# phazei/ComfyUI-HunyuanVideo-Foley

Hardware: AMD Instinct MI355X
Metric: audio-sec/sec (5s clip, 50-step Euler, CFG 4.5) (higher is better)
Workload: dtype bf16; 1 GPU; c2: T2A 5 s, 50 Euler steps, CFG 4.5, hunyuanvideo-foley-xxl, bs=1/GPU, bf16 GEMM operands / fp32 accumulate, weight storage none, DAC-VAE fp32 decode to 48 kHz, host-to-host (H2D noise + D2H waveform timed); clips_per_gpu=1, parallelism=dp1, hip_graph=True, progress_callback=False, collectives=0, bundle_bytes=10565004032, rccl_nranks=1

## Files before the change

comfyui-hunyuanvideo-foley_amd/csrc/foley_rt.hip:

```cpp
#include "../../include/foley_hip.h"
#include "kernels.h"
#include "gemm_plan.h"

#include <algorithm>
#include <climits>
#include <cmath>
#include <cstdio>
#include <cstdlib>
#include <cstring>
#include <cxxabi.h>
#include <atomic>
#include <mutex>
#include <string>
#include <unordered_map>
#include <vector>

thread_local FoleyProfHook g_foley_prof = {nullptr, nullptr};

static std::mutex g_setup_mutex;

static thread_local std::string g_err;
int foley_set_err(const char* msg, const char* file, int line) {
  const char* base = strrchr(file, '/');
  g_err = std::string(msg) + " (" + (base ? base + 1 : file) + ":" + std::to_string(line) + ")";
// ... 699 lines not shown
  RowBcast r{base, ld, 2, rows_per_cfg, L, nullptr, 0, Ls, (float)Ls / (float)L, per, 0, 0};
  if (per > 0) {
    r.dense_from = lead < 0 ? INT_MAX : lead;
    r.dense_base = lead < 0 ? 0 : lead * per;
  }
  return r;
}

static int prof_begin(foley_ctx* c, hipStream_t st, const char* label, double flop, double bytes) {
  if (!c->prof.on) return 0;
  ProfRec r{label, flop, bytes, c->prof.get(), c->prof.get(), nullptr};
  c->prof.recs.push_back(r);
  g_foley_prof = FoleyProfHook{r.e0, r.e1, nullptr};
  return 0;
}
static int prof_end(foley_ctx* c, hipStream_t st) {
  if (!c->prof.on) return 0;
  if (g_foley_prof.e0) {
    g_foley_prof.e0 = nullptr;
    HIPTRY(hipEventRecord(c->prof.recs.back().e0, st));
    HIPTRY(hipEventRecord(c->prof.recs.back().e1, st));
  } else {
    c->prof.recs.back().fn = g_foley_prof.fn;
  }
  return 0;
}
#define PROF(label, flop, bytes, call)            \
  do {                                            \
    TRY(prof_begin(c, st, (label), (flop), (bytes))); \
    TRY(call);                                    \
    TRY(prof_end(c, st));                         \
  } while (0)

static int run_forward(foley_ctx* c, hipStream_t st) {
  const foley_config& f = c->cfg;
  const foley_plan& pl = c->plan;
  const ForwardW& W = c->fw;
  if (!W.ok) return FAIL(FOLEY_ERR_STATE, "forward weights are not resolved (foley_prepare)");
  auto krot = [&pl](GemmArgs g) {
    g.krot_ok = pl.clips == 1 ? 1 : 0;
    return g;
  };
  const int D = f.hidden, H = f.heads, C = f.latent_dim, T = f.compute_dtype;
  const int ncfg = pl.ncfg, clips = pl.clips, La = pl.La, Lv = pl.Lv, Ls = pl.Ls, Lt = pl.Lt, NI = pl.n_iter;
  const int Bc = ncfg * clips, M = Bc * La, Mv = Bc * Lv, S = La + Lv;
  const int th = c->txt_rows ? Bc : ncfg, vh = c->vis_rows ? Bc : ncfg, tdiv = Bc / th, vdiv = Bc / vh;
  const bool bf = foley_is_half(T);
  const size_t es = esize(T);
  const int Sp = (S + 31) & ~31, Lap = (La + 31) & ~31;
  const int* sp = c->step_ctr;
  auto gf = [](double m, double n, double k) { return 2.0 * m * n * k; };
  auto gb = [&](double m, double n, double k, double out_es) { return (m * k + n * k) * (double)es + m * n * out_es; };
  auto af = [&](double b, double sq, double skv) { return 4.0 * b * H * sq * skv * 128.0; };
  auto ab = [&](double b, double sq, double skv) { return (2.0 * b * H * sq * 128.0 + 2.0 * b * H * skv * 128.0) * (double)es; };

  if (!c->smod_hoisted) {
    const int lead = c->sync_per ? c->sync_lead : 0, R = lead * c->sync_per + (vh - lead) * Ls;
    if (c->vis_rows && lead > 1)
      TRY(launch_rows_add_act(c->sync_lead_rows, rb_vec(c->vec_table, D, sp), lead * c->sync_per, D, 1, c->svec, T, st));
    else
      for (int h = 0; h < lead; ++h)
        TRY(launch_rows_add_act(c->sync_tok + (size_t)h * Ls * D, rb_vec(c->vec_table, D, sp), c->sync_per, D, 1,
                                (char*)c->svec + (size_t)h * c->sync_per * D * es, T, st));
    if (lead < vh)
      TRY(launch_rows_add_act(c->sync_tok + (size_t)lead * Ls * D, rb_vec(c->vec_table, D, sp), (vh - lead) * Ls, D, 1,
                              (char*)c->svec + (size_t)lead * c->sync_per * D * es, T, st));
    if (f.depth_single > 0) {
      const double n = (double)f.depth_single * 6 * D;
      GemmArgs gm = krot(gemm_plain(c->svec, R, W.smod, c->smod, (long)f.depth_single * 6 * D));
      PROF("single.modulation (all blocks, one GEMM)", gf(R, n, D), gb(R, n, D, 4), launch_gemm(gm, T, EPI_STORE_F32, 0, st));
    }
  }

  {
    GemmArgs g = krot(gemm_plain(c->xin, M, W.audio_in, c->audio, D));
    g.rb = rb_up(c->sync_tok, D, vdiv * La, La, Ls);
    PROF("audio_embedder", gf(M, D, C), gb(M, D, C, 4), launch_gemm(g, T, EPI_STORE_F32, 0, st));
  }
  if (c->vis_rows)
    TRY(launch_gather_rows(c->v_cond0, c->rep_idx, Bc * Lv, 1, c->vis_src * Lv, D, c->vcond, st));
  else
    TRY(launch_gather_rows(c->v_cond0, c->rep_idx, clips * Lv, ncfg, Lv, D, c->vcond, st));

  LnPending pend[2] = {LnPending{}, LnPending{}};
  const int slab_half = bf ? T : 0;
  auto with_partials = [&](GemmArgs& g, float* slabs) {
    g.partial_half = slab_half ? 1 : 0;
    g.partials = slabs;
    g.partial_stride = (long)g.M * g.N;
    g.partial_cap = PART_CAP;
  };
  const double ln_bytes_t = (double)(M + Mv) * D * (4 + 4 + es), ln_bytes_s = (double)M * D * (4 + 4 + es);
  for (int blk = 0; blk < f.depth_triple; ++blk) {
    const TripleW& w = W.t[blk];
    auto tb = [&](int s, int chunk) {
      return rb_vec(c->modtab + ((size_t)(blk * 2 + s) * NI) * 9 * D + (size_t)chunk * D, 9L * D, sp);
    };
    struct Stream { float* x; void* xn; float* qkv; void* att; void* hid; int rows, L, tok_off; const int* pos; };
    Stream ss[2] = {{c->audio, c->xn_a, c->qkv_a, c->att_a, c->hid_a, M, La, Lv, pl.pos_audio_self},
                    {c->vcond, c->xn_v, c->qkv_v, c->att_v, c->hid_v, Mv, Lv, 0, pl.pos_visual_self}};
    auto ln2 = [&](int c_shift, int c_scale) -> int {
      LnArgs a0{ss[0].x, ss[0].rows, tb(0, c_shift), tb(0, c_scale), ss[0].xn, pend[0]};
      LnArgs a1{ss[1].x, ss[1].rows, tb(1, c_shift), tb(1, c_scale), ss[1].xn, pend[1]};
      pend[0] = pend[1] = LnPending{};
      PROF("triple.layernorm+modulate (+pending split-K sum)", 0.0, ln_bytes_t, launch_ln_mod_pair(a0, a1, D, 1e-6f, T, st));
      return 0;
    };
    auto gated2 = [&](const char* label, const Lin& la, const Lin& lv, bool from_hid, int c_gate) -> int {
      GemmArgs g0 = krot(gemm_plain(from_hid ? ss[0].hid : ss[0].att, ss[0].rows, la, ss[0].x, D));
      GemmArgs g1 = krot(gemm_plain(from_hid ? ss[1].hid : ss[1].att, ss[1].rows, lv, ss[1].x, D));
      g0.rb = tb(0, c_gate);
      g1.rb = tb(1, c_gate);
      with_partials(g0, c->part_a);
      with_partials(g1, c->part_v);
      int ks = 1;
// ... 111 lines not shown
         launch_ln_mod_pending(c->audio, M, D, 1e-5f, sm(3), sm(4), c->xn_a, T, pend[0], st));
    pend[0] = LnPending{};
    PROF("single.w1/w3 conv3 GEMM + SiLU gate", gf(M, 2 * Hc, 3 * D), gb(M, 2 * Hc, 3 * D, es) - (double)M * Hc * es,
         launch_gemm(krot(gemm_conv(c->xn_a, M, La, D, 3, 1, w.w13, c->hid_a, Hc)), T, EPI_SILUGATE_T, 0, st));
    {
      GemmArgs g = krot(gemm_conv(c->hid_a, M, La, Hc, 3, 1, w.w2, c->audio, D));
      g.rb = sm(5);
      with_partials(g, c->part_a);
      int ks = 1;
      PROF("single.w2 conv3 GEMM (gated residual)", gf(M, D, 3 * Hc), gb(M, D, 3 * Hc, 4), launch_gemm(g, T, EPI_GATE_RES, 0, st, &ks));
      if (ks > 1) pend[0] = LnPending{c->part_a, ks, g.partial_stride, w.w2.b, g.rb, slab_half};
    }
  }

  {
    PROF("final.layernorm", 0.0, ln_bytes_s,
         launch_ln_mod_pending(c->audio, M, D, 1e-6f, rb_none(), rb_none(), c->xn_a, T, pend[0], st));
    PROF("final.linear", gf(M, C, D), gb(M, C, D, 4), launch_gemm(krot(gemm_plain(c->xn_a, M, W.fin, c->pred, C)), T, EPI_STORE_F32, 0, st));
  }
  return 0;
}

extern "C" int foley_dit_forward(foley_ctx* c, const float* latents, int iter, float* out_rows, void* stream_v) {
  if (!c || !latents || !out_rows) return FAIL(FOLEY_ERR_INVALID, "null argument");
  if (!c->prepared) return FAIL(FOLEY_ERR_STATE, "foley_prepare has not been called");
  if (iter < 0 || iter >= c->plan.n_iter) return FAIL(FOLEY_ERR_INVALID, "iteration out of range");
  hipStream_t st = (hipStream_t)stream_v;
  HIPTRY(hipSetDevice(c->device));
  const foley_plan& pl = c->plan;
  const int C = c->cfg.latent_dim;
  HIPTRY(hipMemcpyAsync(c->step_ctr, &iter, sizeof(int), hipMemcpyHostToDevice, st));
  HIPTRY(hipStreamSynchronize(st));
  TRY(launch_latent_rows(latents, pl.clips, C, pl.La, pl.ncfg, c->xin, c->cfg.compute_dtype, st));
  TRY(run_forward(c, st));
  HIPTRY(hipMemcpyAsync(out_rows, c->pred, (size_t)pl.ncfg * pl.clips * pl.La * C * 4, hipMemcpyDeviceToDevice, st));
  return 0;
}

extern "C" int foley_profile_forward(foley_ctx* c, const float* latents, int iter, int repeats, foley_prof_entry* out,
                                     int cap, int* n_out, float* bracket_ms, void* stream_v) {
  if (!c || !latents || !out || !n_out || cap < 1 || repeats < 1) return FAIL(FOLEY_ERR_INVALID, "bad argument");
  if (!c->prepared) return FAIL(FOLEY_ERR_STATE, "foley_prepare has not been called");
  if (iter < 0 || iter >= c->plan.n_iter) return FAIL(FOLEY_ERR_INVALID, "iteration out of range");
  hipStream_t st = (hipStream_t)stream_v;
  HIPTRY(hipSetDevice(c->device));
  const foley_plan& pl = c->plan;
  HIPTRY(hipMemcpyAsync(c->step_ctr, &iter, sizeof(int), hipMemcpyHostToDevice, st));
  HIPTRY(hipStreamSynchronize(st));
  TRY(launch_latent_rows(latents, pl.clips, c->cfg.latent_dim, pl.La, pl.ncfg, c->xin, c->cfg.compute_dtype, st));
  TRY(run_forward(c, st));
  c->prof.recs.clear();
  c->prof.used = 0;
  c->prof.on = true;
  int rc = 0;
  for (int r = 0; r < repeats && rc == 0; ++r) rc = run_forward(c, st);
  c->prof.on = false;
  g_foley_prof = FoleyProfHook{nullptr, nullptr, nullptr};
  if (rc) return rc;
  constexpr int NCAL = 32;
  hipEvent_t cal[2 * NCAL];
  for (int i = 0; i < 2 * NCAL; ++i) cal[i] = c->prof.get();
  for (int i = 0; i < NCAL; ++i) {
    HIPTRY(hipEventRecord(cal[2 * i], st));
    HIPTRY(hipEventRecord(cal[2 * i + 1], st));
  }
  HIPTRY(hipStreamSynchronize(st));
  double cal_ms = 0.0;
  for (int i = 0; i < NCAL; ++i) {
    float ms = 0.f;
    HIPTRY(hipEventElapsedTime(&ms, cal[2 * i], cal[2 * i + 1]));
    cal_ms += ms;
  }
  if (bracket_ms) *bracket_ms = (float)(cal_ms / NCAL);
  int n = 0;
  for (const ProfRec& r : c->prof.recs) {
    float ms = 0.f;
    HIPTRY(hipEventElapsedTime(&ms, r.e0, r.e1));
    int j = 0;
    for (; j < n; ++j)
      if (!strcmp(out[j].label, r.label)) break;
    if (j == n) {
      if (n == cap) return FAIL(FOLEY_ERR_INVALID, "profile: entry buffer too small");
      memset(&out[n], 0, sizeof(out[n]));
      strncpy(out[n].label, r.label, sizeof(out[n].label) - 1);
      if (r.fn) {
        const char* mangled = hipKernelNameRefByPtr(r.fn, st);
        if (mangled) {
          int status = 0;
          char* dm = abi::__cxa_demangle(mangled, nullptr, nullptr, &status);
          strncpy(out[n].kernel, status == 0 && dm ? dm : mangled, sizeof(out[n].kernel) - 1);
          free(dm);
        }
      }
      ++n;
    }
    out[j].calls += 1;
    out[j].total_ms += ms;
    out[j].flop += r.flop;
    out[j].bytes += r.bytes;
  }
  *n_out = n;
  return 0;
}

static int run_iteration(foley_ctx* c, hipStream_t st) {
  const foley_plan& pl = c->plan;
  TRY(run_forward(c, st));
  StepArgs s{};
  s.pred = c->pred; s.x = c->x_cur; s.x_saved = c->x_saved; s.d_acc = c->d_acc;
  s.clips = pl.clips; s.C = c->cfg.latent_dim; s.L = pl.La; s.ncfg = pl.ncfg;
  s.guidance = pl.guidance; s.coef = pl.solver_coef; s.step_ptr = c->step_ctr;
  s.rows_out = c->xin; s.rows_dtype = c->cfg.compute_dtype;
  if (c->edit) {
    StepEditArgs e{};
    e.s = s;
    e.x0 = (const float*)c->edit_x0.p; e.noise = (const float*)c->edit_noise.p;
    e.mask = c->edit_mask_clips ? (const float*)c->edit_mask.p : nullptr;
    e.x0_clips = c->edit_x0_clips; e.mask_clips = c->edit_mask_clips;
    return launch_solver_step_edit(e, st);
  }
  return launch_solver_step(s, st);
}

static int edit_key(const foley_ctx* c) {
  if (!c->edit) return 0;
  return 1 | (c->edit_x0_clips == 1 ? 2 : 0) | (c->edit_mask_clips ? 4 : 0) | (c->edit_mask_clips == 1 ? 8 : 0);
}

extern "C" int foley_set_edit(foley_ctx* c, const float* x0, int x0_clips, const float* noise, const float* mask, int mask_clips,
                              void* stream_v) {
  if (!c) return FAIL(FOLEY_ERR_INVALID, "null context");
  if (!c->prepared) return FAIL(FOLEY_ERR_STATE, "foley_set_edit: foley_prepare has not been called");
  if (!x0 && !noise && !mask) {
    c->edit = false;
    return 0;
  }
  if (!x0 || !noise) return FAIL(FOLEY_ERR_INVALID, "foley_set_edit: x0 and noise are required (all three null clears the edit state)");
  const foley_plan& pl = c->plan;
  if (x0_clips != 1 && x0_clips != pl.clips) return FAIL(FOLEY_ERR_INVALID, "foley_set_edit: x0_clips must be 1 or the plan's clips");
  if (mask && mask_clips != 1 && mask_clips != pl.clips)
    return FAIL(FOLEY_ERR_INVALID, "foley_set_edit: mask_clips must be 1 or the plan's clips");
  std::lock_guard<std::mutex> setup_lock(g_setup_mutex);
  hipStream_t st = (hipStream_t)stream_v;
  HIPTRY(hipSetDevice(c->device));
  HIPTRY(hipStreamSynchronize(st));
// ... 15 lines not shown
extern "C" int foley_sample(foley_ctx* c, float* latents, int use_graph, foley_progress_cb cb, void* user,
                            void* stream_v) {
  if (!c || !latents) return FAIL(FOLEY_ERR_INVALID, "null argument");
  if (!c->prepared) return FAIL(FOLEY_ERR_STATE, "foley_prepare has not been called");
  hipStream_t st = (hipStream_t)stream_v;
  HIPTRY(hipSetDevice(c->device));
  const foley_plan& pl = c->plan;
  const size_t xbytes = (size_t)pl.clips * c->cfg.latent_dim * pl.La * 4;
  if (c->graph_exec && c->graph_key != edit_key(c)) ctx_drop_graph(c);
  if (use_graph && !c->graph_exec) {
    std::lock_guard<std::mutex> setup_lock(g_setup_mutex);
    hipStream_t cs;
    HIPTRY(hipStreamSynchronize(st));
    HIPTRY(hipStreamCreateWithFlags(&cs, hipStreamNonBlocking));
    hipGraph_t graph = nullptr;
    hipError_t e = hipStreamBeginCapture(cs, hipStreamCaptureModeThreadLocal);
    int rc = 0;
    if (e == hipSuccess) {
      rc = run_iteration(c, cs);
      hipError_t e2 = hipStreamEndCapture(cs, &graph);
      if (e == hipSuccess) e = e2;
    }
    if (e == hipSuccess && rc == 0) e = hipGraphInstantiate(&c->graph_exec, graph, nullptr, nullptr, 0);
    if (graph) (void)hipGraphDestroy(graph);
    (void)hipStreamDestroy(cs);
    if (rc != 0) return rc;
    if (e != hipSuccess) return FAIL(FOLEY_ERR_HIP, hipGetErrorString(e));
    c->graph_guidance = pl.guidance;
    c->graph_key = edit_key(c);
  }
  c->abort_req.store(0, std::memory_order_relaxed);
  HIPTRY(hipEventRecord(c->ev0, st));
  HIPTRY(hipMemcpyAsync(c->x_cur, latents, xbytes, hipMemcpyDeviceToDevice, st));
  HIPTRY(hipMemsetAsync(c->step_ctr, 0, sizeof(int), st));
  TRY(launch_latent_rows(c->x_cur, pl.clips, c->cfg.latent_dim, pl.La, pl.ncfg, c->xin, c->cfg.compute_dtype, st));
  for (int it = 0; it < pl.n_iter; ++it) {
    if (use_graph) HIPTRY(hipGraphLaunch(c->graph_exec, st));
    else TRY(run_iteration(c, st));
    if (cb) {
      HIPTRY(hipMemcpyAsync(latents, c->x_cur, xbytes, hipMemcpyDeviceToDevice, st));
      HIPTRY(hipStreamSynchronize(st));
      cb(it + 1, pl.n_iter, user);
    }
    if (c->abort_req.exchange(0, std::memory_order_acq_rel)) {
      if (!cb) {
        HIPTRY(hipMemcpyAsync(latents, c->x_cur, xbytes, hipMemcpyDeviceToDevice, st));
        HIPTRY(hipStreamSynchronize(st));
      }
      return FAIL(FOLEY_ERR_ABORTED, "sampling loop aborted by foley_abort()");
    }
  }
  HIPTRY(hipMemcpyAsync(latents, c->x_cur, xbytes, hipMemcpyDeviceToDevice, st));
  HIPTRY(hipEventRecord(c->ev1, st));
  c->timed = true;
  return 0;
}

extern "C" int foley_abort(foley_ctx* c) {
  if (!c) return FAIL(FOLEY_ERR_INVALID, "null context");
  c->abort_req.store(1, std::memory_order_release);
  return 0;
}

extern "C" int foley_dac_decode(foley_ctx* c, const float* latents, int clips, int T, float* wave, void* stream_v) {
  if (!c || !latents || !wave || clips < 1 || T < 1) return FAIL(FOLEY_ERR_INVALID, "bad argument");
  hipStream_t st = (hipStream_t)stream_v;
  HIPTRY(hipSetDevice(c->device));
  const foley_config& f = c->cfg;
// ... 356 lines not shown
  for (int i = 0; i < 2; ++i) {
    if (a[i].M < 0) return FAIL(FOLEY_ERR_INVALID, "ln_mod pair: negative row count");
    if (!parts[i]) continue;
    if (ks[i] < 1 || !gate[i]) return FAIL(FOLEY_ERR_INVALID, "pending split-K: partials, k >= 1 and a gate are required");
    if (pdt[i] != 0 && pdt[i] != out_dtype) return FAIL(FOLEY_ERR_INVALID, "pending split-K: 16-bit slabs must have the output dtype");
    a[i].pend = LnPending{(const float*)parts[i], ks[i], (long)a[i].M * D, bias[i], to_rb(gate[i]), pdt[i]};
  }
  return launch_ln_mod_pair(a[0], a[1], D, eps, out_dtype, (hipStream_t)stream);
}

extern "C" int foley_op_ln_mod_pending(float* x, int M, int D, float eps, const foley_rowbcast* shift,
                                       const foley_rowbcast* scale, void* out, int out_dtype, const float* partials,
                                       int k, const float* bias, const foley_rowbcast* gate, void* stream) {
  return foley_op_ln_mod_pending2(x, M, D, eps, shift, scale, out, out_dtype, partials, 0, k, bias, gate, stream);
}

extern "C" int foley_op_qkv_split(const float* qkv, int M, int L, int H, int nK, const float* const* gain,
                                  const int32_t* const* pos, void* const* dst, int out_dtype, int vt_pitch,
                                  int S_tot, int tok_off, float eps, const float* cos_tab, const float* sin_tab,
                                  void* stream) {
  if (nK < 1 || nK > 3) return FAIL(FOLEY_ERR_INVALID, "nK must be 1..3");
  QkvSplitArgs a{};
  a.qkv = qkv; a.M = M; a.L = L; a.H = H; a.nK = nK;
  for (int i = 0; i < nK; ++i) {
    a.gain[i] = gain ? gain[i] : nullptr;
    a.pos[i] = pos ? pos[i] : nullptr;
    a.dst[i] = dst[i];
  }
  a.out_dtype = out_dtype; a.vt_pitch = vt_pitch;
  a.S_tot = S_tot; a.tok_off = tok_off; a.eps = eps; a.cos_tab = cos_tab; a.sin_tab = sin_tab;
  return launch_qkv_split(a, (hipStream_t)stream);
}

extern "C" int foley_op_solver_step(const float* pred, float* x, float* x_saved, float* d_acc, int clips, int C,
                                    int L, int ncfg, float guidance, const float* coef, int32_t* step_ptr,
                                    void* rows_out, int rows_dtype, void* stream) {
  StepArgs s{pred, x, x_saved, d_acc, clips, C, L, ncfg, guidance, coef, step_ptr, rows_out, rows_dtype};
  return launch_solver_step(s, (hipStream_t)stream);
}

extern "C" int foley_op_solver_step_edit(const float* pred, float* x, float* x_saved, float* d_acc, int clips, int C, int L,
                                         int ncfg, float guidance, const float* coef, int32_t* step_ptr, void* rows_out,
                                         int rows_dtype, const float* x0, int x0_clips, const float* noise, const float* mask,
                                         int mask_clips, void* stream) {
  StepEditArgs e{};
  e.s = StepArgs{pred, x, x_saved, d_acc, clips, C, L, ncfg, guidance, coef, step_ptr, rows_out, rows_dtype};
  e.x0 = x0; e.noise = noise; e.mask = mask; e.x0_clips = x0_clips; e.mask_clips = mask_clips;
  return launch_solver_step_edit(e, (hipStream_t)stream);
}

extern "C" int foley_op_flow_mix(const float* noise, const float* x0, int x0_clips, int clips, int C, int L, float sigma,
                                 float* out, void* stream) {
  return launch_flow_mix(noise, x0, x0_clips, clips, C, L, sigma, out, (hipStream_t)stream);
}

extern "C" int foley_op_latent_rows(const float* x, int clips, int C, int L, int ncfg, void* out, int out_dtype,
                                    void* stream) {
  return launch_latent_rows(x, clips, C, L, ncfg, out, out_dtype, (hipStream_t)stream);
}

extern "C" int foley_op_dac_out(const float* s, const float* w, const float* bias, int B, int T, int C, float* out,
                                void* stream) {
  return launch_dac_out(s, w, bias, B, T, C, out, (hipStream_t)stream);
}
```

comfyui-hunyuanvideo-foley_amd/csrc/kernels.h:

```cpp
#pragma once
#include "common.h"

enum GemmEpi {
  EPI_STORE_F32 = 0,
  EPI_STORE_T = 1,
  EPI_SILU_T = 2,
  EPI_GELU_T = 3,
  EPI_SILUGATE_T = 4,
  EPI_GATE_RES = 5,
  EPI_DAC = 6,
  EPI_QKV_SPLIT = 7,
  EPI_QKV_ATTN = 8,
  EPI_COUNT
};

struct QkvSplitArgs {
  const float* qkv;
  int M, L, H, nK;
  const float* gain[3];
  const int* pos[3];
  void* dst[3];
  int S_tot, tok_off;
  int out_dtype;
  int vt_pitch;
// ... 78 lines not shown
  const float* partials;
  int k;
  long stride;
  const float* bias;
  RowBcast gate;
  int half;
};
struct LnArgs {
  float* x;
  int M;
  RowBcast shift, scale;
  void* out;
  LnPending pend;
};
int launch_ln_mod_pending(float* x, int M, int D, float eps, const RowBcast& shift, const RowBcast& scale,
                          void* out, int out_dtype, const LnPending& pend, hipStream_t st);
int launch_ln_mod_pair(const LnArgs& a0, const LnArgs& a1, int D, float eps, int out_dtype, hipStream_t st);

int launch_qkv_split(const QkvSplitArgs& a, hipStream_t st);
int launch_qkv_split_pair(const QkvSplitArgs& a0, const QkvSplitArgs& a1, hipStream_t st);

int launch_rows_add_act(const float* a, const RowBcast& v, int R, int D, int act_silu, void* out,
                        int out_dtype, hipStream_t st);
int launch_rows_periodic_check(const float* x, int groups, int rows, int period, int D, int* flag, hipStream_t st);
int launch_add_periodic(const float* x, const float* pos, int R, int D, int period, void* out,
                        int out_dtype, hipStream_t st);
int launch_gather_rows(const float* src, const int* idx, int n_idx, int groups, int src_rows, int D,
                       float* out, hipStream_t st);
int launch_cast(const void* src, int src_dtype, void* dst, int dst_dtype, long n, hipStream_t st);

int launch_latent_rows(const float* x, int clips, int C, int L, int ncfg, void* out, int out_dtype,
                       hipStream_t st);

struct StepArgs {
  const float* pred;
  float* x;
  float* x_saved;
  float* d_acc;
  int clips, C, L, ncfg;
  float guidance;
  const float* coef;
  int* step_ptr;
  void* rows_out;
  int rows_dtype;
};
int launch_solver_step(const StepArgs& a, hipStream_t st);
struct StepEditArgs {
  StepArgs s;
  const float* x0;
  const float* noise;
  const float* mask;
  int x0_clips, mask_clips;
};
int launch_solver_step_edit(const StepEditArgs& a, hipStream_t st);
int launch_flow_mix(const float* noise, const float* x0, int x0_clips, int clips, int C, int L, float sigma, float* out,
                    hipStream_t st);

int launch_dac_in(const float* x, const float* w, const float* bias, const float* alpha, int B, int T, int C,
                  float* out0, float* out1, hipStream_t st);
int launch_rows_to_planes(const float* rows, int B, int T, int C, float* out, hipStream_t st);
int launch_qkv_regroup(const void* qkv, int n_rows, int dtype, int H, const int* idx_q, int G, int Sq, const int* idx_kv, int Skv, void* q, void* k,
                       void* v, int vt_pitch, hipStream_t st);
int launch_resize_aa_u8(const uint8_t* in, long outer, int len_in, long inner, int len_out, const int* xmin, const int* xsize,
                        const short* w, int kmax, int prec, uint8_t* out, hipStream_t st);
int launch_resample_sinc(const float* x, int B, int N, int orig, int nnew, const float* taps, int ntaps, int width, float* out,
                         int Nout, hipStream_t st);
int launch_logmel(const float* w16, int B, int N16, const float* basis, const int* mel_lo, const int* mel_len, const float* mel_w,
                  int mel_wp, void* patches, int out_dtype, float* mel_out, hipStream_t st);
int launch_dac_out(const float* s, const float* w, const float* bias, int B, int T, int C, float* out,
                   hipStream_t st);
```

comfyui-hunyuanvideo-foley_amd/csrc/rowops.hip:

```cpp
#include <type_traits>

#include "kernels.h"

namespace {

#define FOLEY_LAUNCH_CHECK()                                                             \
  do {                                                                                   \
    hipError_t _e = hipGetLastError();                                                   \
    if (_e != hipSuccess) return foley_set_err(hipGetErrorString(_e), __FILE__, __LINE__); \
  } while (0)

template <typename OutT> struct Pack4;
template <> struct Pack4<float> {
  static __device__ __forceinline__ void store(float* p, const f32x4 v) { *(f32x4*)p = v; }
};
template <> struct Pack4<bf16_t> {
  static __device__ __forceinline__ void store(bf16_t* p, const f32x4 v) {
    uint2 w;
    w.x = pack_bf16x2(v[0], v[1]);
    w.y = pack_bf16x2(v[2], v[3]);
    *(uint2*)p = w;
  }
};

template <> struct Pack4<f16_t> {
  static __device__ __forceinline__ void store(f16_t* p, const f32x4 v) {
    uint2 w;
    w.x = pack_f16x2(v[0], v[1]);
    w.y = pack_f16x2(v[2], v[3]);
    *(uint2*)p = w;
  }
};
// ... 353 lines not shown
    out[i] = src[((long)g * src_rows + idx[l]) * D + c];
  }
}

template <typename S, typename Dst>
__global__ void cast_kernel(const S* __restrict__ s, Dst* __restrict__ d, long n) {
  for (long i = (long)blockIdx.x * blockDim.x + threadIdx.x; i < n; i += (long)gridDim.x * blockDim.x)
    d[i] = Cvt<Dst>::to(Cvt<S>::from(s[i]));
}

template <typename OutT>
__global__ __launch_bounds__(256) void latent_rows_kernel(const float* __restrict__ x, int clips, int C, int L,
                                                          int ncfg, OutT* __restrict__ out) {
  __shared__ float tile[32][33];
  const int b = blockIdx.z;
  const int l0 = blockIdx.x * 32, c0 = blockIdx.y * 32;
  const int tx = threadIdx.x & 31, ty = threadIdx.x >> 5;
  for (int i = ty; i < 32; i += 8) {
    const int c = c0 + i, l = l0 + tx;
    tile[i][tx] = (c < C && l < L) ? x[((long)b * C + c) * L + l] : 0.f;
  }
  __syncthreads();
  for (int i = ty; i < 32; i += 8) {
    const int l = l0 + i, c = c0 + tx;
    if (l < L && c < C) {
      const OutT v = Cvt<OutT>::to(tile[tx][i]);
      for (int g = 0; g < ncfg; ++g) out[(((long)g * clips + b) * L + l) * C + c] = v;
    }
  }
}

constexpr int STEP_SAVE_X = 1, STEP_USE_SAVED = 2, STEP_ACC_RESET = 4;

template <typename OutT>
__global__ __launch_bounds__(256) void solver_step_kernel(const StepArgs a) {
  __shared__ float tile[32][33];
  const int it = *a.step_ptr;
  const float* cf = a.coef + (long)it * 8;
  const float w_new = cf[0], w_acc = cf[1], dt = cf[2], w_store = cf[3];
  const int flags = (int)cf[4];
  const int b = blockIdx.z;
  const int l0 = blockIdx.x * 32, c0 = blockIdx.y * 32;
  const int tx = threadIdx.x & 31, ty = threadIdx.x >> 5;
  const long rows = (long)a.clips * a.L;
  for (int i = ty; i < 32; i += 8) {
    const int l = l0 + i, c = c0 + tx;
    float v = 0.f;
    if (l < a.L && c < a.C) {
      const long r = (long)b * a.L + l;
      if (a.ncfg == 2) {
        const float u = a.pred[r * a.C + c], cnd = a.pred[(rows + r) * a.C + c];
        v = u + a.guidance * (cnd - u);
      } else {
        v = a.pred[r * a.C + c];
      }
    }
    tile[i][tx] = v;
  }
  __syncthreads();
  for (int i = ty; i < 32; i += 8) {
    const int c = c0 + i, l = l0 + tx;
    float xn = 0.f;
    if (c < a.C && l < a.L) {
      const long xi = ((long)b * a.C + c) * a.L + l;
      const float v = tile[tx][i];
      const float xc = a.x[xi];
      float acc = 0.f;
      if (a.d_acc) acc = (flags & STEP_ACC_RESET) ? 0.f : a.d_acc[xi];
      const float deriv = (w_acc != 0.f) ? (w_new * v + w_acc * acc) : (w_new * v);
      const float base = (flags & STEP_USE_SAVED) ? a.x_saved[xi] : xc;
      if (flags & STEP_SAVE_X) a.x_saved[xi] = xc;
      xn = base + deriv * dt;
      a.x[xi] = xn;
      if (a.d_acc) a.d_acc[xi] = acc + w_store * v;
    }
    tile[tx][i] = xn;
  }
  __syncthreads();
  if (a.rows_out) {
    for (int i = ty; i < 32; i += 8) {
      const int l = l0 + i, c = c0 + tx;
      if (l < a.L && c < a.C) {
        const OutT v = Cvt<OutT>::to(tile[i][tx]);
        for (int g = 0; g < a.ncfg; ++g)
          ((OutT*)a.rows_out)[(((long)g * a.clips + b) * a.L + l) * a.C + c] = v;
      }
    }
  }
}

constexpr int STEP_BLEND = 8;

template <typename OutT>
__global__ __launch_bounds__(256) void solver_step_edit_kernel(const StepEditArgs e) {
  __shared__ float tile[32][33];
  const StepArgs& a = e.s;
  const int it = *a.step_ptr;
  const float* cf = a.coef + (long)it * 8;
  const float w_new = cf[0], w_acc = cf[1], dt = cf[2], w_store = cf[3];
  const int flags = (int)cf[4];
  const float s_next = cf[5];
  const int b = blockIdx.z;
  const int l0 = blockIdx.x * 32, c0 = blockIdx.y * 32;
  const int tx = threadIdx.x & 31, ty = threadIdx.x >> 5;
  const long rows = (long)a.clips * a.L;
  for (int i = ty; i < 32; i += 8) {
    const int l = l0 + i, c = c0 + tx;
    float v = 0.f;
    if (l < a.L && c < a.C) {
      const long r = (long)b * a.L + l;
      if (a.ncfg == 2) {
        const float u = a.pred[r * a.C + c], cnd = a.pred[(rows + r) * a.C + c];
        v = u + a.guidance * (cnd - u);
      } else {
        v = a.pred[r * a.C + c];
      }
    }
    tile[i][tx] = v;
  }
  __syncthreads();
  const float* x0b = e.x0 + (e.x0_clips == 1 ? 0L : (long)b * a.C * a.L);
  const float* mb = e.mask ? e.mask + (e.mask_clips == 1 ? 0L : (long)b * a.L) : nullptr;
  for (int i = ty; i < 32; i += 8) {
    const int c = c0 + i, l = l0 + tx;
    float xn = 0.f;
    if (c < a.C && l < a.L) {
      const long xi = ((long)b * a.C + c) * a.L + l;
      const float v = tile[tx][i];
      const float xc = a.x[xi];
      float acc = 0.f;
      if (a.d_acc) acc = (flags & STEP_ACC_RESET) ? 0.f : a.d_acc[xi];
      const float deriv = (w_acc != 0.f) ? (w_new * v + w_acc * acc) : (w_new * v);
      const float base = (flags & STEP_USE_SAVED) ? a.x_saved[xi] : xc;
      if (flags & STEP_SAVE_X) a.x_saved[xi] = xc;
      xn = base + deriv * dt;
      if (flags & STEP_BLEND) {
        const float m = mb ? mb[l] : 1.f;
        const float tgt = s_next * e.noise[xi] + (1.f - s_next) * x0b[(long)c * a.L + l];
        xn = m * xn + (1.f - m) * tgt;
      }
      a.x[xi] = xn;
      if (a.d_acc) a.d_acc[xi] = acc + w_store * v;
    }
    tile[tx][i] = xn;
  }
  __syncthreads();
  if (a.rows_out) {
    for (int i = ty; i < 32; i += 8) {
      const int l = l0 + i, c = c0 + tx;
      if (l < a.L && c < a.C) {
        const OutT v = Cvt<OutT>::to(tile[i][tx]);
        for (int g = 0; g < a.ncfg; ++g)
          ((OutT*)a.rows_out)[(((long)g * a.clips + b) * a.L + l) * a.C + c] = v;
      }
    }
  }
}

__global__ __launch_bounds__(256) void flow_mix_kernel(const float* __restrict__ noise, const float* __restrict__ x0,
                                                       long plane, long n, int x0_per_clip, float sigma,
                                                       float* __restrict__ out) {
  const long i = (long)blockIdx.x * 256 + threadIdx.x;
  if (i >= n) return;
  const float src = x0[x0_per_clip ? i : i % plane];
  out[i] = sigma * noise[i] + (1.f - sigma) * src;
}

__global__ void step_increment_kernel(int* p) { *p = *p + 1; }

__global__ __launch_bounds__(256) void dac_out_kernel(const float* __restrict__ s, const float* __restrict__ w,
                                                      const float* __restrict__ bias, int T, int C,
                                                      float* __restrict__ out) {
  extern __shared__ float sm[];
  const int b = blockIdx.y;
  const int t0 = blockIdx.x * 64;
  const int pitch = C + 1;
  float* rows = sm;
  float* wl = sm + 70 * pitch;
  for (int i = threadIdx.x; i < 7 * C; i += 256) wl[i] = w[i];
  for (int i = threadIdx.x; i < 70 * C; i += 256) {
    const int rr = i / C, c = i - rr * C;
    const int t = t0 + rr - 3;
    rows[rr * pitch + c] = (t >= 0 && t < T) ? s[((long)b * T + t) * C + c] : 0.f;
  }
  __syncthreads();
  const int ti = threadIdx.x >> 2, part = threadIdx.x & 3;
  const int cq = C >> 2;
  float acc = 0.f;
  for (int j = 0; j < 7; ++j) {
    const float* rp = rows + (ti + j) * pitch + part * cq;
    const float* wp = wl + j * C + part * cq;
    for (int c = 0; c < cq; ++c) acc += rp[c] * wp[c];
  }
  acc += __shfl_xor(acc, 1, 64);
  acc += __shfl_xor(acc, 2, 64);
  const int t = t0 + ti;
  if (part == 0 && t < T) out[(long)b * T + t] = tanhf(acc + bias[0]);
}

__global__ __launch_bounds__(256) void dac_in_kernel(const float* __restrict__ x, const float* __restrict__ w,
                                                     const float* __restrict__ bias, const float* __restrict__ alpha,
// ... 218 lines not shown
  return 0;
}

int launch_cast(const void* src, int sd, void* dst, int dd, long n, hipStream_t st) {
  dim3 g(grid1d(n, 256)), b(256);
  if (sd == FOLEY_F32 && dd == FOLEY_BF16)
    FOLEY_LAUNCH((cast_kernel<float, bf16_t>), g, b, 0, st, (const float*)src, (bf16_t*)dst, n);
  else if (sd == FOLEY_BF16 && dd == FOLEY_F32)
    FOLEY_LAUNCH((cast_kernel<bf16_t, float>), g, b, 0, st, (const bf16_t*)src, (float*)dst, n);
  else if (sd == FOLEY_F32 && dd == FOLEY_F16)
    FOLEY_LAUNCH((cast_kernel<float, f16_t>), g, b, 0, st, (const float*)src, (f16_t*)dst, n);
  else if (sd == FOLEY_F16 && dd == FOLEY_F32)
    FOLEY_LAUNCH((cast_kernel<f16_t, float>), g, b, 0, st, (const f16_t*)src, (float*)dst, n);
  else if (sd == FOLEY_F32 && dd == FOLEY_F32)
    FOLEY_LAUNCH((cast_kernel<float, float>), g, b, 0, st, (const float*)src, (float*)dst, n);
  else return foley_set_err("cast: unsupported dtype pair", __FILE__, __LINE__);
  FOLEY_LAUNCH_CHECK();
  return 0;
}

int launch_latent_rows(const float* x, int clips, int C, int L, int ncfg, void* out, int out_dtype, hipStream_t st) {
  dim3 grid((L + 31) / 32, (C + 31) / 32, clips), block(256);
  if (out_dtype == FOLEY_F32)
    FOLEY_LAUNCH(latent_rows_kernel<float>, grid, block, 0, st, x, clips, C, L, ncfg, (float*)out);
  else if (out_dtype == FOLEY_BF16)
    FOLEY_LAUNCH(latent_rows_kernel<bf16_t>, grid, block, 0, st, x, clips, C, L, ncfg, (bf16_t*)out);
  else if (out_dtype == FOLEY_F16)
    FOLEY_LAUNCH(latent_rows_kernel<f16_t>, grid, block, 0, st, x, clips, C, L, ncfg, (f16_t*)out);
  else return foley_set_err("latent_rows: bad dtype", __FILE__, __LINE__);
  FOLEY_LAUNCH_CHECK();
  return 0;
}

int launch_solver_step(const StepArgs& a, hipStream_t st) {
  dim3 grid((a.L + 31) / 32, (a.C + 31) / 32, a.clips), block(256);
  if (a.rows_dtype == FOLEY_BF16) FOLEY_LAUNCH(solver_step_kernel<bf16_t>, grid, block, 0, st, a);
  else if (a.rows_dtype == FOLEY_F16) FOLEY_LAUNCH(solver_step_kernel<f16_t>, grid, block, 0, st, a);
  else FOLEY_LAUNCH(solver_step_kernel<float>, grid, block, 0, st, a);
  FOLEY_LAUNCH_CHECK();
  FOLEY_LAUNCH(step_increment_kernel, dim3(1), dim3(1), 0, st, a.step_ptr);
  FOLEY_LAUNCH_CHECK();
  return 0;
}

int launch_solver_step_edit(const StepEditArgs& e, hipStream_t st) {
  const StepArgs& a = e.s;
  if (!e.x0 || !e.noise) return foley_set_err("solver_step_edit: x0 and noise are required", __FILE__, __LINE__);
  if ((e.x0_clips != 1 && e.x0_clips != a.clips) || (e.mask && e.mask_clips != 1 && e.mask_clips != a.clips))
    return foley_set_err("solver_step_edit: x0 / mask clip count must be 1 or clips", __FILE__, __LINE__);
  dim3 grid((a.L + 31) / 32, (a.C + 31) / 32, a.clips), block(256);
  if (a.rows_dtype == FOLEY_BF16) FOLEY_LAUNCH(solver_step_edit_kernel<bf16_t>, grid, block, 0, st, e);
  else if (a.rows_dtype == FOLEY_F16) FOLEY_LAUNCH(solver_step_edit_kernel<f16_t>, grid, block, 0, st, e);
  else FOLEY_LAUNCH(solver_step_edit_kernel<float>, grid, block, 0, st, e);
  FOLEY_LAUNCH_CHECK();
  FOLEY_LAUNCH(step_increment_kernel, dim3(1), dim3(1), 0, st, a.step_ptr);
  FOLEY_LAUNCH_CHECK();
  return 0;
}

int launch_flow_mix(const float* noise, const float* x0, int x0_clips, int clips, int C, int L, float sigma, float* out,
                    hipStream_t st) {
  if (!noise || !x0 || !out || clips < 1 || C < 1 || L < 1 || (x0_clips != 1 && x0_clips != clips))
    return foley_set_err("flow_mix: bad arguments (x0 clip count must be 1 or clips)", __FILE__, __LINE__);
  const long plane = (long)C * L, n = plane * clips;
  FOLEY_LAUNCH(flow_mix_kernel, dim3(grid1d(n, 256)), dim3(256), 0, st, noise, x0, plane, n, x0_clips != 1 || clips == 1 ? 1 : 0,
               sigma, out);
  FOLEY_LAUNCH_CHECK();
  return 0;
}

int launch_dac_in(const float* x, const float* w, const float* bias, const float* alpha, int B, int T, int C,
                  float* out0, float* out1, hipStream_t st) {
  if (C % 4) return foley_set_err("dac_in: channel count must be a multiple of 4", __FILE__, __LINE__);
  FOLEY_LAUNCH(dac_in_kernel, dim3(grid1d((long)B * T * (C / 4), 256)), dim3(256), 0, st, x, w, bias, alpha, B, T, C,
                     out0, out1);
  FOLEY_LAUNCH_CHECK();
  return 0;
}

template <typename E>
__global__ __launch_bounds__(256) void qkv_regroup_kernel(const E* __restrict__ qkv, int H, const int* __restrict__ idx_q, int Sq,
                                                          const int* __restrict__ idx_kv, int Skv, E* __restrict__ q, E* __restrict__ k,
                                                          E* __restrict__ v, int vt_pitch, int n_rows) {
  constexpr int HD = 64, CPR = HD * sizeof(E) / 16;
  __shared__ __attribute__((aligned(16))) E tile[64][HD + 16 / sizeof(E)];
  const int t0 = blockIdx.x * 64, h = blockIdx.y, g = blockIdx.z;
  const long ld = 3L * H * HD;
  const int tid = threadIdx.x;
// ... 127 lines not shown
```

Measured before the change: 14.15 audio-sec/sec.

## Fold step-counter increment and vcond gather into solver step kernel

Removes the separate single-thread step_increment kernel: the last solver-step block, detected through an atomic ticket counter, advances the step pointer. The per-iteration visual-condition row gather moves out of the forward pass into extra z-slices of the solver step kernel, so it stages the next iteration's vcond rows. Each iteration drops two kernel launches in the graph. In exchange it adds an atomic ticket word and a dependence on grid-wide last-block completion ordering, and the gather now overlaps with the solver work.

Result: no change. 14.15 audio-sec/sec, median of 3 (-0.0%).

```diff
diff --git a/comfyui-hunyuanvideo-foley_amd/csrc/foley_rt.hip b/comfyui-hunyuanvideo-foley_amd/csrc/foley_rt.hip
--- a/comfyui-hunyuanvideo-foley_amd/csrc/foley_rt.hip
+++ b/comfyui-hunyuanvideo-foley_amd/csrc/foley_rt.hip
@@ -755,6 +755,17 @@
     TRY(prof_end(c, st));                         \
   } while (0)
 
+static StageRows vcond_rows(const foley_ctx* c) {
+  const foley_plan& pl = c->plan;
+  const int D = c->cfg.hidden;
+  if (c->vis_rows) return StageRows{c->v_cond0, c->rep_idx, pl.ncfg * pl.clips * pl.Lv, 1, c->vis_src * pl.Lv, D, c->vcond};
+  return StageRows{c->v_cond0, c->rep_idx, pl.clips * pl.Lv, pl.ncfg, pl.Lv, D, c->vcond};
+}
+static int stage_vcond(foley_ctx* c, hipStream_t st) {
+  const StageRows g = vcond_rows(c);
+  return launch_gather_rows(g.src, g.idx, g.n_idx, g.groups, g.src_rows, g.D, g.out, st);
+}
+
 static int run_forward(foley_ctx* c, hipStream_t st) {
   const foley_config& f = c->cfg;
   const foley_plan& pl = c->plan;
@@ -800,10 +811,6 @@
     g.rb = rb_up(c->sync_tok, D, vdiv * La, La, Ls);
     PROF("audio_embedder", gf(M, D, C), gb(M, D, C, 4), launch_gemm(g, T, EPI_STORE_F32, 0, st));
   }
-  if (c->vis_rows)
-    TRY(launch_gather_rows(c->v_cond0, c->rep_idx, Bc * Lv, 1, c->vis_src * Lv, D, c->vcond, st));
-  else
-    TRY(launch_gather_rows(c->v_cond0, c->rep_idx, clips * Lv, ncfg, Lv, D, c->vcond, st));
 
   LnPending pend[2] = {LnPending{}, LnPending{}};
   const int slab_half = bf ? T : 0;
@@ -981,6 +988,7 @@
   HIPTRY(hipMemcpyAsync(c->step_ctr, &iter, sizeof(int), hipMemcpyHostToDevice, st));
   HIPTRY(hipStreamSynchronize(st));
   TRY(launch_latent_rows(latents, pl.clips, C, pl.La, pl.ncfg, c->xin, c->cfg.compute_dtype, st));
+  TRY(stage_vcond(c, st));
   TRY(run_forward(c, st));
   HIPTRY(hipMemcpyAsync(out_rows, c->pred, (size_t)pl.ncfg * pl.clips * pl.La * C * 4, hipMemcpyDeviceToDevice, st));
   return 0;
@@ -997,12 +1005,16 @@
   HIPTRY(hipMemcpyAsync(c->step_ctr, &iter, sizeof(int), hipMemcpyHostToDevice, st));
   HIPTRY(hipStreamSynchronize(st));
   TRY(launch_latent_rows(latents, pl.clips, c->cfg.latent_dim, pl.La, pl.ncfg, c->xin, c->cfg.compute_dtype, st));
+  TRY(stage_vcond(c, st));
   TRY(run_forward(c, st));
   c->prof.recs.clear();
   c->prof.used = 0;
   c->prof.on = true;
   int rc = 0;
-  for (int r = 0; r < repeats && rc == 0; ++r) rc = run_forward(c, st);
+  for (int r = 0; r < repeats && rc == 0; ++r) {
+    rc = stage_vcond(c, st);
+    if (rc == 0) rc = run_forward(c, st);
+  }
   c->prof.on = false;
   g_foley_prof = FoleyProfHook{nullptr, nullptr, nullptr};
   if (rc) return rc;
@@ -1058,8 +1070,9 @@
   StepArgs s{};
   s.pred = c->pred; s.x = c->x_cur; s.x_saved = c->x_saved; s.d_acc = c->d_acc;
   s.clips = pl.clips; s.C = c->cfg.latent_dim; s.L = pl.La; s.ncfg = pl.ncfg;
-  s.guidance = pl.guidance; s.coef = pl.solver_coef; s.step_ptr = c->step_ctr;
+  s.guidance = pl.guidance; s.coef = pl.solver_coef; s.step_ptr = c->step_ctr; s.ticket = (unsigned*)c->step_ctr + 1;
   s.rows_out = c->xin; s.rows_dtype = c->cfg.compute_dtype;
+  s.stage = vcond_rows(c);
   if (c->edit) {
     StepEditArgs e{};
     e.s = s;
@@ -1141,8 +1154,9 @@
   c->abort_req.store(0, std::memory_order_relaxed);
   HIPTRY(hipEventRecord(c->ev0, st));
   HIPTRY(hipMemcpyAsync(c->x_cur, latents, xbytes, hipMemcpyDeviceToDevice, st));
-  HIPTRY(hipMemsetAsync(c->step_ctr, 0, sizeof(int), st));
+  HIPTRY(hipMemsetAsync(c->step_ctr, 0, 2 * sizeof(int), st));
   TRY(launch_latent_rows(c->x_cur, pl.clips, c->cfg.latent_dim, pl.La, pl.ncfg, c->xin, c->cfg.compute_dtype, st));
+  TRY(stage_vcond(c, st));
   for (int it = 0; it < pl.n_iter; ++it) {
     if (use_graph) HIPTRY(hipGraphLaunch(c->graph_exec, st));
     else TRY(run_iteration(c, st));
@@ -1565,10 +1579,20 @@
   return launch_qkv_split(a, (hipStream_t)stream);
 }
 
+__device__ unsigned g_op_step_ticket;
+static int op_step_args(StepArgs* s, void* rows_out, int rows_dtype, int32_t* step_ptr) {
+  void* t = nullptr;
+  HIPTRY(hipGetSymbolAddress(&t, HIP_SYMBOL(g_op_step_ticket)));
+  s->step_ptr = step_ptr; s->ticket = (unsigned*)t;
+  s->rows_out = rows_out; s->rows_dtype = rows_dtype;
+  return 0;
+}
+
 extern "C" int foley_op_solver_step(const float* pred, float* x, float* x_saved, float* d_acc, int clips, int C,
                                     int L, int ncfg, float guidance, const float* coef, int32_t* step_ptr,
                                     void* rows_out, int rows_dtype, void* stream) {
-  StepArgs s{pred, x, x_saved, d_acc, clips, C, L, ncfg, guidance, coef, step_ptr, rows_out, rows_dtype};
+  StepArgs s{pred, x, x_saved, d_acc, clips, C, L, ncfg, guidance, coef};
+  TRY(op_step_args(&s, rows_out, rows_dtype, step_ptr));
   return launch_solver_step(s, (hipStream_t)stream);
 }
 
@@ -1577,7 +1601,8 @@
                                          int rows_dtype, const float* x0, int x0_clips, const float* noise, const float* mask,
                                          int mask_clips, void* stream) {
   StepEditArgs e{};
-  e.s = StepArgs{pred, x, x_saved, d_acc, clips, C, L, ncfg, guidance, coef, step_ptr, rows_out, rows_dtype};
+  e.s = StepArgs{pred, x, x_saved, d_acc, clips, C, L, ncfg, guidance, coef};
+  TRY(op_step_args(&e.s, rows_out, rows_dtype, step_ptr));
   e.x0 = x0; e.noise = noise; e.mask = mask; e.x0_clips = x0_clips; e.mask_clips = mask_clips;
   return launch_solver_step_edit(e, (hipStream_t)stream);
 }
diff --git a/comfyui-hunyuanvideo-foley_amd/csrc/kernels.h b/comfyui-hunyuanvideo-foley_amd/csrc/kernels.h
--- a/comfyui-hunyuanvideo-foley_amd/csrc/kernels.h
+++ b/comfyui-hunyuanvideo-foley_amd/csrc/kernels.h
@@ -134,6 +134,12 @@
 int launch_latent_rows(const float* x, int clips, int C, int L, int ncfg, void* out, int out_dtype,
                        hipStream_t st);
 
+struct StageRows {
+  const float* src;
+  const int* idx;
+  int n_idx, groups, src_rows, D;
+  float* out;
+};
 struct StepArgs {
   const float* pred;
   float* x;
@@ -143,8 +149,10 @@
   float guidance;
   const float* coef;
   int* step_ptr;
+  unsigned* ticket;
   void* rows_out;
   int rows_dtype;
+  StageRows stage;
 };
 int launch_solver_step(const StepArgs& a, hipStream_t st);
 struct StepEditArgs {
diff --git a/comfyui-hunyuanvideo-foley_amd/csrc/rowops.hip b/comfyui-hunyuanvideo-foley_amd/csrc/rowops.hip
--- a/comfyui-hunyuanvideo-foley_amd/csrc/rowops.hip
+++ b/comfyui-hunyuanvideo-foley_amd/csrc/rowops.hip
@@ -1,3 +1,4 @@
+#include <algorithm>
 #include <type_traits>
 
 #include "kernels.h"
@@ -417,10 +418,41 @@
 
 constexpr int STEP_SAVE_X = 1, STEP_USE_SAVED = 2, STEP_ACC_RESET = 4;
 
+__device__ __forceinline__ int step_read(const StepArgs& a, int* lds_it) {
+  if (threadIdx.x == 0) *lds_it = *a.step_ptr;
+  __syncthreads();
+  return *lds_it;
+}
+
+__device__ __forceinline__ void step_advance(const StepArgs& a, int it) {
+  if (threadIdx.x != 0) return;
+  const unsigned n = gridDim.x * gridDim.y * (unsigned)a.clips;
+  if (atomicAdd(a.ticket, 1u) == n - 1) {
+    *a.ticket = 0u;
+    *a.step_ptr = it + 1;
+  }
+}
+
+__device__ __forceinline__ void step_stage_rows(const StepArgs& a) {
+  const StageRows& g = a.stage;
+  const int D4 = g.D >> 2;
+  const long n4 = (long)g.groups * g.n_idx * D4;
+  const long nthr = (long)(gridDim.z - a.clips) * gridDim.y * gridDim.x * 256;
+  const long t0 = ((((long)blockIdx.z - a.clips) * gridDim.y + blockIdx.y) * gridDim.x + blockIdx.x) * 256 + threadIdx.x;
+  for (long i = t0; i < n4; i += nthr) {
+    const long r = i / D4;
+    const int c = (int)(i - r * D4);
+    const int grp = (int)(r / g.n_idx), l = (int)(r - (long)grp * g.n_idx);
+    ((float4*)g.out)[i] = ((const float4*)g.src)[((long)grp * g.src_rows + g.idx[l]) * D4 + c];
+  }
+}
+
 template <typename OutT>
 __global__ __launch_bounds__(256) void solver_step_kernel(const StepArgs a) {
   __shared__ float tile[32][33];
-  const int it = *a.step_ptr;
+  __shared__ int lds_it;
+  if ((int)blockIdx.z >= a.clips) return step_stage_rows(a);
+  const int it = step_read(a, &lds_it);
   const float* cf = a.coef + (long)it * 8;
   const float w_new = cf[0], w_acc = cf[1], dt = cf[2], w_store = cf[3];
   const int flags = (int)cf[4];
@@ -472,6 +504,7 @@
       }
     }
   }
+  step_advance(a, it);
 }
 
 constexpr int STEP_BLEND = 8;
@@ -479,8 +512,10 @@
 template <typename OutT>
 __global__ __launch_bounds__(256) void solver_step_edit_kernel(const StepEditArgs e) {
   __shared__ float tile[32][33];
+  __shared__ int lds_it;
   const StepArgs& a = e.s;
-  const int it = *a.step_ptr;
+  if ((int)blockIdx.z >= a.clips) return step_stage_rows(a);
+  const int it = step_read(a, &lds_it);
   const float* cf = a.coef + (long)it * 8;
   const float w_new = cf[0], w_acc = cf[1], dt = cf[2], w_store = cf[3];
   const int flags = (int)cf[4];
@@ -540,6 +575,7 @@
       }
     }
   }
+  step_advance(a, it);
 }
 
 __global__ __launch_bounds__(256) void flow_mix_kernel(const float* __restrict__ noise, const float* __restrict__ x0,
@@ -550,8 +586,6 @@
   const float src = x0[x0_per_clip ? i : i % plane];
   out[i] = sigma * noise[i] + (1.f - sigma) * src;
 }
-
-__global__ void step_increment_kernel(int* p) { *p = *p + 1; }
 
 __global__ __launch_bounds__(256) void dac_out_kernel(const float* __restrict__ s, const float* __restrict__ w,
                                                       const float* __restrict__ bias, int T, int C,
@@ -836,13 +870,25 @@
   return 0;
 }
 
+static int step_grid(const StepArgs& a, dim3* grid) {
+  if (!a.ticket) return foley_set_err("solver_step: a ticket word is required", __FILE__, __LINE__);
+  *grid = dim3((a.L + 31) / 32, (a.C + 31) / 32, a.clips);
+  const StageRows& g = a.stage;
+  if (!g.src) return 0;
+  if (!g.idx || !g.out || g.n_idx < 1 || g.groups < 1 || g.D < 4 || (g.D & 3))
+    return foley_set_err("solver_step: staged rows need an index, an output and a row length that is a multiple of 4", __FILE__, __LINE__);
+  const long n4 = (long)g.groups * g.n_idx * (g.D >> 2), per_z = (long)grid->x * grid->y;
+  const long blocks = std::min<long>((n4 + 511) / 512, 256);
+  grid->z += (unsigned)((blocks + per_z - 1) / per_z);
+  return 0;
+}
+
 int launch_solver_step(const StepArgs& a, hipStream_t st) {
-  dim3 grid((a.L + 31) / 32, (a.C + 31) / 32, a.clips), block(256);
+  dim3 grid, block(256);
+  if (int rc = step_grid(a, &grid)) return rc;
   if (a.rows_dtype == FOLEY_BF16) FOLEY_LAUNCH(solver_step_kernel<bf16_t>, grid, block, 0, st, a);
   else if (a.rows_dtype == FOLEY_F16) FOLEY_LAUNCH(solver_step_kernel<f16_t>, grid, block, 0, st, a);
   else FOLEY_LAUNCH(solver_step_kernel<float>, grid, block, 0, st, a);
-  FOLEY_LAUNCH_CHECK();
-  FOLEY_LAUNCH(step_increment_kernel, dim3(1), dim3(1), 0, st, a.step_ptr);
   FOLEY_LAUNCH_CHECK();
   return 0;
 }
@@ -852,12 +898,11 @@
   if (!e.x0 || !e.noise) return foley_set_err("solver_step_edit: x0 and noise are required", __FILE__, __LINE__);
   if ((e.x0_clips != 1 && e.x0_clips != a.clips) || (e.mask && e.mask_clips != 1 && e.mask_clips != a.clips))
     return foley_set_err("solver_step_edit: x0 / mask clip count must be 1 or clips", __FILE__, __LINE__);
-  dim3 grid((a.L + 31) / 32, (a.C + 31) / 32, a.clips), block(256);
+  dim3 grid, block(256);
+  if (int rc = step_grid(a, &grid)) return rc;
   if (a.rows_dtype == FOLEY_BF16) FOLEY_LAUNCH(solver_step_edit_kernel<bf16_t>, grid, block, 0, st, e);
   else if (a.rows_dtype == FOLEY_F16) FOLEY_LAUNCH(solver_step_edit_kernel<f16_t>, grid, block, 0, st, e);
   else FOLEY_LAUNCH(solver_step_edit_kernel<float>, grid, block, 0, st, e);
-  FOLEY_LAUNCH_CHECK();
-  FOLEY_LAUNCH(step_increment_kernel, dim3(1), dim3(1), 0, st, a.step_ptr);
   FOLEY_LAUNCH_CHECK();
   return 0;
 }
```
